# sajadn/Exemplar-VAE

Measured on AMD Instinct MI355X. Metric: training images/sec, higher is better.
Workload: dtype f32

## Files before the change

exemplar-vae_amd/csrc/evae_dense.hip:

```cpp

#include "evae_gemm_x6.h"
#include "evae_gemm_p6.h"
#include "evae_thin.h"
#include "evae_u8_prepare.h"

namespace evae {

__global__ void gated_bwd_input_kernel(const float* __restrict__ dout, const float* __restrict__ gout,
                                       const float* __restrict__ s, int M, int N, int ldo,
                                       float* __restrict__ dh, float* __restrict__ dg, int ldd) {
  const size_t n = (size_t)M * N;
  size_t i = (size_t)blockIdx.x * blockDim.x + threadIdx.x;
  const size_t stride = (size_t)gridDim.x * blockDim.x;
  for (; i < n; i += stride) {
    const size_t row = i / N, col = i % N;
    const float d = dout[row * (size_t)ldd + col], ov = gout[i], sv = s[i];
    const size_t o = row * (size_t)ldo + col;
    dh[o] = d * sv;
    dg[o] = d * ov * (1.0f - sv);
  }
}

__global__ __launch_bounds__(256) void gated_bwd_input_v4_kernel(const float4* __restrict__ dout, const float4* __restrict__ gout,
                                                                 const float4* __restrict__ s, unsigned nquads, unsigned nq,
// ... 953 lines not shown
  const bool narrow = gemm_x6_pick_bn(M, K) == 64;
  if (u8_img) {
    if (narrow) return launch_gemm_p6<EPI_GATE_BWD_IMG, 64, true>(g, 1, stream, "dense_bwd_data(p6, gate, byte-layer images)");
    return launch_gemm_p6<EPI_GATE_BWD_IMG, 128, true>(g, 1, stream, "dense_bwd_data(p6, gate, byte-layer images)");
  }
  if (gate) {
    if (narrow) return launch_gemm_p6<EPI_GATE_BWD, 64, true>(g, 1, stream, "dense_bwd_data(p6, gate)");
    return launch_gemm_p6<EPI_GATE_BWD, 128, true>(g, 1, stream, "dense_bwd_data(p6, gate)");
  }
  if (narrow) return launch_gemm_p6<EPI_LINEAR, 64, true>(g, 1, stream, "dense_bwd_data(p6)");
  return launch_gemm_p6<EPI_LINEAR, 128, true>(g, 1, stream, "dense_bwd_data(p6)");
}

struct P6WgradPlan { int kc, nz, ksplit, local; };
static P6WgradPlan p6_wgrad_plan(int nks, int N, int K, bool with_db) {
  P6WgradPlan p;
  p.kc = K + (with_db ? 1 : 0);
  const int tiles = cdiv(N, BM) * cdiv(p.kc, 64);
  static int slots = -1, local = -1;
  if (slots < 0) { const char* e = getenv("EVAE_P6_WGRAD_SLOTS"); slots = e ? atoi(e) : 256; }
  if (local < 0) { const char* e = getenv("EVAE_P6_WGRAD_LOCAL"); local = e ? atoi(e) : 16; }
  int nz = std::max(1, std::min(slots / std::max(tiles, 1), nks / 8));
  p.local = 0;
  if (local >= 8 && nz >= 8) {
    const int want = (local >= 16 && tiles * 2 <= 64 && nks / 16 >= 8) ? 16 : 8;
    if (tiles * (want / 8) <= 64) { nz = want; p.local = 1; }
  }
  p.ksplit = cdiv(nks, nz);
  p.nz = cdiv(nks, p.ksplit);
  return p;
}
extern "C" size_t evae_dense_bwd_weight_p6_workspace_bytes(int nks, int N, int K) {
  if (nks <= 0 || N <= 0 || K <= 0) return 256;
  const P6WgradPlan p = p6_wgrad_plan(nks, N, K, true);
  return align_up((size_t)p.nz * N * p.kc * sizeof(float), 256) + 256;
}
extern "C" int evae_dense_bwd_weight_p6(const void* dyT_img, const void* xT_img, int nks, int N, int K, float* dw, float* db,
                                        void* ws, size_t ws_bytes, evae_stream_t stream_) {
  EVAE_REQUIRE(nks > 0 && N > 0 && K > 0 && dyT_img && xT_img && dw, "dense_bwd_weight_p6: bad arguments");
  const P6WgradPlan p = p6_wgrad_plan(nks, N, K, db != nullptr);
  if (ws == nullptr || ws_bytes < (size_t)p.nz * N * p.kc * sizeof(float)) { set_error("dense_bwd_weight_p6: workspace too small (%zu)", ws_bytes); return EVAE_EWORKSPACE; }
  hipStream_t stream = (hipStream_t)stream_;
  GemmArgs g = {};
  g.ones_col = -1; g.npairs = 1;
  g.A[0] = (const float*)dyT_img; g.B[0] = (const float*)xT_img; g.Kc[0] = nks * P6_KS; g.M = N; g.N = p.kc;
  g.out0 = (float*)ws; g.ldo = p.kc; g.ksplit = p.ksplit; g.sk_local = p.local ? p.nz : 0;
  int rc = launch_gemm_p6<EPI_RAW, 64>(g, p.nz, stream, "dense_bwd_weight(p6)");
  if (rc) return rc;
  FinishArgs f = {};
  f.part = (const float*)ws; f.nz = p.nz; f.M = N; f.N = p.kc; f.ldo = p.kc; f.epi = EPI_RAW; f.out0 = dw;
  f.ones_col = db ? K : -1; f.out_db = db;
  return launch_finish(f, stream);
}
```

exemplar-vae_amd/csrc/evae_gemm_p6.h:

```cpp
#pragma once
#include "evae_gemm_kernel.h"

namespace evae {

typedef __bf16 p6_bf16x8 __attribute__((ext_vector_type(8)));
typedef __bf16 p6_bf16x4 __attribute__((ext_vector_type(4)));
typedef __attribute__((address_space(3))) void* p6_lds_t;
typedef __attribute__((address_space(3))) p6_bf16x4* p6_lds4_t;

constexpr int P6_NS = 3;
constexpr int p6_stage_bytes(int bn) { return P6_TILE + 3 * bn * 32; }
constexpr int p6_lds_bytes(int bn) { return P6_NS * p6_stage_bytes(bn); }

typedef unsigned p6_u32x2 __attribute__((ext_vector_type(2)));
template <int OFF>
__device__ __forceinline__ p6_u32x2 p6_tr_read(unsigned lds_addr) {
  p6_u32x2 r;
  asm volatile("ds_read_b64_tr_b16 %0, %1 offset:%2" : "=v"(r) : "v"(lds_addr), "n"(OFF));
  return r;
}

template <int EPI, int BN_, bool TA = false>
__global__ __launch_bounds__(256) __attribute__((amdgpu_waves_per_eu(2, 2))) void gemm_p6_kernel(const GemmArgs g) {
  constexpr bool GATED = (EPI == EPI_GATED || EPI == EPI_RAW_GATED);
  static_assert(BN_ == 128 || (BN_ == 64 && !GATED), "column tile: 128, or 64 for narrow plain outputs");
  constexpr int NW = 4, MT = 2, NT = BN_ / 64;
  constexpr int SB = p6_stage_bytes(BN_), BOFF = P6_TILE, BPL = BN_ * 32;
  extern __shared__ __attribute__((aligned(16))) float smem[];
  char* const lds = reinterpret_cast<char*>(smem);
  const int ntiles = g.tiles_m * g.tiles_n;
  int tile, zs = blockIdx.z;
  if (g.sk_local > 0) {
    const int id = blockIdx.x, xcd = id & 7, slot = id >> 3;
    const int j = slot / ntiles;
    tile = slot - j * ntiles;
    zs = xcd + 8 * j;
    if (zs >= g.sk_local) return;
  } else {
    const int id = blockIdx.x, xcd = id & 7, slot = id >> 3;
    const int qq = ntiles >> 3, rr = ntiles & 7;
    tile = (xcd < rr ? xcd * (qq + 1) : rr * (qq + 1) + (xcd - rr) * qq) + slot;
  }
  const int tm = tile / g.tiles_n, tn = tile - tm * g.tiles_n;
  const int m0 = tm * BM;
  const int n0 = GATED ? tn * 64 : tn * BN_;
  const int tid = threadIdx.x, lane = tid & 63;
  const int wave = __builtin_amdgcn_readfirstlane(tid >> 6);
  const int wr = wave >> 1, wc = wave & 1, l31 = lane & 31, lh = lane >> 5;

  f32x16 acc[MT][NT];
#pragma unroll
  for (int i = 0; i < MT; ++i)
#pragma unroll
    for (int j = 0; j < NT; ++j)
#pragma unroll
      for (int r = 0; r < 16; ++r) acc[i][j][r] = 0.f;

  const int nks = g.Kc[0] / P6_KS;
  int s_begin = 0, s_end = nks;
  if (g.ksplit > 0) {
    s_begin = zs * g.ksplit;
    const int e = s_begin + g.ksplit;
    if (e < s_end) s_end = e;
  }
  const int nst = s_end - s_begin;

  const unsigned a_nms = TA ? (unsigned)g.lda[0] : 0u;
  const unsigned grp = (unsigned)nks * P6_GROUP;
  const char* const abase = reinterpret_cast<const char*>(g.A[0]) + (TA ? (size_t)tm * 8 * P6_GROUP : (size_t)tm * 8 * grp);
  const char* const bbase = reinterpret_cast<const char*>(g.B[0]) + (size_t)(GATED ? tn * 8 : tn * (BN_ / 16)) * grp;
  const rsrc_t rA = make_rsrc(abase, 0x7FFFFFFFu);
  const rsrc_t rB = make_rsrc(bbase, 0x7FFFFFFFu);
  const unsigned voff_a = TA ? 0u : (unsigned)lh * grp + (unsigned)l31 * 16u;
  const unsigned voff_b = (unsigned)lh * grp + (unsigned)l31 * 16u;
  const unsigned voff_ta = (unsigned)lh * P6_GROUP + (unsigned)((((l31 >> 1) ^ (4 * lh)) * 32) + (l31 & 1) * 16);

  constexpr int NPIECE = BN_ == 128 ? 6 : 5;
  auto issue_piece = [&](int ks, int b, int q) {
    const unsigned so = (unsigned)ks * (unsigned)P6_GROUP;
    char* const st = lds + b * SB;
    if (q < 3) {
      if constexpr (TA) {
        __builtin_amdgcn_raw_ptr_buffer_load_lds(rA, (p6_lds_t)(st + q * P6_PLANE + wave * 1024), 16, voff_ta,
                                                 (unsigned)ks * a_nms * (unsigned)P6_GROUP + wave * 2 * P6_GROUP + q * P6_CHUNK, 0, 0);
      } else {
        __builtin_amdgcn_raw_ptr_buffer_load_lds(rA, (p6_lds_t)(st + q * P6_PLANE + wave * 1024), 16, voff_a,
                                                 so + (unsigned)(2 * wave) * grp + q * P6_CHUNK, 0, 0);
      }
    } else if constexpr (BN_ == 128) {
      const int p = q - 3;
      __builtin_amdgcn_raw_ptr_buffer_load_lds(rB, (p6_lds_t)(st + BOFF + p * BPL + wave * 1024), 16, voff_b,
                                               so + (unsigned)(2 * wave) * grp + p * P6_CHUNK, 0, 0);
// ... 109 lines not shown
            EVAE_P6_SB;
          }
          if constexpr (ISSUE) {
            constexpr int stride = NMF / 6;
            if (j % stride == 1 && j / stride < NPIECE) issue_piece(s_begin + i + 3, bcur, j / stride);
            EVAE_P6_SB;
          }
        }
    __builtin_amdgcn_s_setprio(0);
  };
#undef EVAE_P6_SB

  constexpr std::integral_constant<int, 0> I0{};
  constexpr std::integral_constant<int, 1> I1{};
  constexpr std::integral_constant<int, 2> I2{};
  constexpr std::true_type T{};
  constexpr std::false_type F{};
  if (nst > 0) {
    issue(s_begin, 0);
    if (nst > 1) issue(s_begin + 1, 1);
    if (nst > 2) issue(s_begin + 2, 2);
    if (nst > 2) wait_steps(I2); else if (nst > 1) wait_steps(I1); else wait_steps(I0);
    __builtin_amdgcn_s_barrier();
    read_all(I0, 0);
    int i = 0, b = 0;
    auto adv = [&]() { ++i; b = b == P6_NS - 1 ? 0 : b + 1; };
    while (i + 4 < nst) {
      iter(I0, T, T, I1, i, b); adv();
      iter(I1, T, T, I1, i, b); adv();
    }
#pragma unroll
    for (int u = 0; u < 2; ++u) {
      if (i < nst) {
        if (i + 3 < nst) iter(I0, T, T, I1, i, b);
        else if (i + 2 < nst) iter(I0, T, F, I1, i, b);
        else if (i + 1 < nst) iter(I0, T, F, I0, i, b);
        else iter(I0, F, F, I0, i, b);
        adv();
      }
      if (i < nst) {
        if (i + 3 < nst) iter(I1, T, T, I1, i, b);
        else if (i + 2 < nst) iter(I1, T, F, I1, i, b);
        else if (i + 1 < nst) iter(I1, T, F, I0, i, b);
        else iter(I1, F, F, I0, i, b);
        adv();
      }
    }
    __syncthreads();
  }
  if (g.dbg == 4) return;
  gemm_epilogue<EPI, BN_, NW, 0>(g, acc, m0, n0, tm, wr, wc, lane, smem, zs);
}

static __global__ __launch_bounds__(256) void p6_pack_rows_kernel(const float* __restrict__ x, const float* __restrict__ x2, int R, int K,
                                                           long long ld, int gated, int rows_img, int nks, unsigned char* __restrict__ img) {
  p6_pack_rows_element((size_t)blockIdx.x * blockDim.x + threadIdx.x, x, x2, R, K, ld, gated, rows_img, nks, img);
}

static __global__ __launch_bounds__(256) void p6_pack_cols_kernel(const float* __restrict__ x, const float* __restrict__ x2, int Kd, int R,
                                                           long long ld, int ones_row, int rows_img, int nks, unsigned char* __restrict__ img) {
  p6_pack_cols_element((size_t)blockIdx.x * blockDim.x + threadIdx.x, x, x2, Kd, R, ld, ones_row, rows_img, nks, img);
}

template <int EPI, int BN_ = 128, bool TA = false>
static int launch_gemm_p6(GemmArgs& g, int nz, hipStream_t stream, const char* what) {
  static bool attr_done = false;
  if (!attr_done) {
    (void)hipFuncSetAttribute((const void*)gemm_p6_kernel<EPI, BN_, TA>, hipFuncAttributeMaxDynamicSharedMemorySize, p6_lds_bytes(BN_));
    attr_done = true;
  }
  constexpr bool GATED = (EPI == EPI_GATED || EPI == EPI_RAW_GATED);
  g.tiles_m = cdiv(g.M, BM);
  g.tiles_n = cdiv(g.N, GATED ? 64 : BN_);
  dim3 grid(g.tiles_m * g.tiles_n, 1, nz);
  if (g.sk_local > 0) {
    if (g.sk_local != nz || g.ksplit <= 0) { set_error("%s: XCD-local split needs sk_local == nz and a split contraction", what); return EVAE_EINVAL; }
    grid = dim3(8 * cdiv(nz, 8) * g.tiles_m * g.tiles_n, 1, 1);
  }
  gemm_p6_kernel<EPI, BN_, TA><<<grid, 256, p6_lds_bytes(BN_), stream>>>(g);
  return check_launch(what);
}

}
```

exemplar-vae_amd/evae/_lib.py:

```python
import ctypes as C
import os

_HERE = os.path.dirname(os.path.abspath(__file__))
LIB_PATH = os.environ.get("EVAE_LIB_PATH") or os.path.join(os.path.dirname(_HERE), "csrc", "libevae_hip.so")

_p = C.c_void_p
_i = C.c_int
_f = C.c_float
_d = C.c_double
_z = C.c_size_t
_l = C.c_int64
_u = C.c_uint


class ConvDesc(C.Structure):
    _fields_ = [(n, C.c_int) for n in ("N", "C", "H", "W", "Co", "KH", "KW", "stride", "pad")]


class WtJob(C.Structure):
    _fields_ = [("w1", C.c_void_p), ("w2", C.c_void_p), ("dst", C.c_void_p), ("N", C.c_int), ("K", C.c_int), ("ldt", C.c_int)]


class CtlJob(C.Structure):
    _fields_ = [("stage0", C.c_void_p), ("stage1", C.c_void_p), ("ctl", C.c_void_p), ("bytes", C.c_size_t), ("state", C.c_void_p),
# ... 45 lines not shown
    "evae_mixture_lse_fwd_workspace_bytes": (_z, [_i, _i, _i]),
    "evae_mixture_lse_fwd": (_i, [_p, _i, _p, _p, _i, _i, _f, _p, _p, _p, _p, _z, _p]),
    "evae_mixture_lse_bwd_workspace_bytes": (_z, [_i, _i, _i]),
    "evae_mixture_lse_bwd": (_i, [_p, _i, _p, _p, _i, _i, _p, _p, _p, _p, _p, _p, _z, _p]),
    "evae_pseudo_inputs_fwd": (_i, [_p, _i, _i, _p, _p]),
    "evae_pseudo_inputs_bwd": (_i, [_p, _p, _i, _i, _p, _p]),
    "evae_pairdist_topk_workspace_bytes": (_z, [_i, _i, _i, _i]),
    "evae_pairdist_topk": (_i, [_p, _i, _p, _i, _i, _i, _u, _l, _p, _p, _p, _z, _p]),
    "evae_pairwise_distance": (_i, [_p, _i, _p, _i, _i, _p, _p]),
    "evae_topk_merge": (_i, [_p, _p, _i, _i, _i, _p, _p, _p]),
    "evae_select_exemplars": (_i, [_p, _i, _p, _i, _p, _p, _p, _p]),
    "evae_dense_fwd_workspace_bytes": (_z, [_i, _i, _i, _i]),
    "evae_gated_dense_fwd": (_i, [_p, _p, _i, _i, _i, _p, _p, _p, _p, _i, _p, _p, _p, _p, _z, _p]),
    "evae_linear_fwd": (_i, [_p, _p, _i, _i, _i, _p, _p, _i, _i, _f, _f, _p, _p, _p, _z, _p]),
    "evae_heads_reparam_fwd_workspace_bytes": (_z, [_i, _i, _i]),
    "evae_heads_reparam_fwd": (_i, [_p, _i, _i, _i, _p, _p, _p, _p, _i, _f, _f, _p, _p, _p, _p, _p, _p, _p, _z, _p]),
    "evae_heads_reparam_fwd_bcast_applies": (_i, [_i, _i, _i, _i]),
    "evae_heads_reparam_fwd_bcast": (_i, [_p, _i, _i, _i, _p, _p, _p, _p, _i, _f, _f, _p, _p, _p, _p, _p, _p, _p, _p, _i, _p]),
    "evae_heads_density_fwd": (_i, [_p, _i, _i, _i, _p, _p, _p, _p, _i, _f, _f, _p, _p, _p, _p, _p, _p, _z, _p]),
    "evae_log_normal_diag_bwd_hardtanh": (_i, [_p, _p, _p, _p, _f, _f, _p, _i, _i, _p, _p, _p, _p]),
    "evae_dense_bwd_data_wt_bytes": (_z, [_i, _i, _i]),
    "evae_dense_bwd_data_wt_ld": (_i, [_i]),
    "evae_dense_bwd_data_wt": (_i, [_p, _p, _p, _p, _i, _i, _i, _i, _p, _p, _p, _p, _i, _p, _p, _z, _p]),
    "evae_dense_bwd_data_workspace_bytes": (_z, [_i, _i, _i, _i]),
    "evae_dense_bwd_data": (_i, [_p, _p, _p, _p, _i, _i, _i, _i, _p, _p, _p, _p, _i, _p, _z, _p]),
    "evae_dense_bwd_weight_workspace_bytes": (_z, [_i, _i, _i]),
    "evae_dense_bwd_weight": (_i, [_p, _i, _i, _i, _p, _p, _i, _i, _p, _p, _i, _p, _z, _p]),
    "evae_dense_bwd_weight_phased": (_i, [_p, _i, _i, _i, _p, _p, _i, _i, _p, _p, _i, _p, _z, _i, _p]),
    "evae_dense_u8_supported": (_i, [_i, C.c_longlong]),
    "evae_dense_u8_prepared_bytes": (_z, [_i, _i]),
    "evae_dense_u8_prepare": (_i, [_p, _p, _i, _i, _p, _z, _p]),
    "evae_gated_dense_fwd_u8": (_i, [_p, _p, _i, _i, C.c_longlong, _f, _p, _p, _p, _i, _p, _p, _p]),
    "evae_dense_bwd_weight_u8_workspace_bytes": (_z, [_i, _i, _i]),
    "evae_dense_bwd_weight_u8": (_i, [_p, _i, _i, C.c_longlong, _p, _p, _i, C.c_longlong, _f, _p, _p, _p, _z, _p]),
    "evae_dense_bwd_weight_u8_phased": (_i, [_p, _i, _i, C.c_longlong, _p, _p, _i, C.c_longlong, _f, _p, _p, _p, _z, _i, _p]),
    "evae_dense_bwd_weight_u8_images": (_i, [_i, _i, _i, C.POINTER(C.c_size_t), C.POINTER(C.c_int)]),
    "evae_broadcast_scalar": (_i, [_p, _p, _i, _p]),
    "evae_sum_small": (_i, [_p, _i, _p, _p]),
    "evae_thin_configure": (_i, [_i]),
    "evae_p6_nks": (_i, [_i]),
    "evae_p6_nks_rows": (_i, [_i]),
    "evae_p6_image_bytes": (_z, [_i, _i]),
    "evae_gemm_p6_applies": (_i, [_i, _i, _i]),
    "evae_p6_pack_rows": (_i, [_p, _p, _i, _i, C.c_longlong, _i, _p, _z, _p]),
    "evae_p6_pack_cols": (_i, [_p, _p, _i, _i, C.c_longlong, _i, _i, _p, _z, _p]),
    "evae_p6_fill_row": (_i, [_p, _i, _i, _f, _i, _i, _p]),
    "evae_gated_dense_fwd_timg": (_i, [_p, _p, _i, _i, _i, _p, _p, _p, _p, _i, _p, _p, _p, _p, _i, _i, _i, _p, _z, _p]),
    "evae_gated_dense_fwd_u8_timg": (_i, [_p, _p, _i, _i, C.c_longlong, _f, _p, _p, _p, _i, _p, _p, _p, _i, _i, _i, _p]),
    "evae_dense_bwd_data_timg": (_i, [_p, _p, _p, _p, _i, _i, _i, _i, _p, _p, _p, _p, _i, _p, _p, _i, _i, _i, _p, _z, _p]),
    "evae_gated_dense_fwd_p6t": (_i, [_p, _i, _i, _i, _p, _p, _p, _i, _p, _p, _p]),
    "evae_dense_bwd_data_p6t": (_i, [_p, _i, _i, _i, _p, _i, _p, _p, _p, _p, _i, _p, _i, _i, _p]),
    "evae_dense_bwd_weight_p6_workspace_bytes": (_z, [_i, _i, _i]),
    "evae_dense_bwd_weight_p6": (_i, [_p, _p, _i, _i, _i, _p, _p, _p, _z, _p]),
    "evae_dense_bwd_data_img": (_i, [_p, _p, _p, _p, _i, _i, _i, _i, _p, _p, _p, _i, _i, _p, _p, _z, _p]),
    "evae_dense_bwd_weight_group": (_i, [_p, _i, _p]),
    "evae_dense_bwd_weight_finish_group": (_i, [_p, _i, _p]),
    "evae_gated_dense_bwd_input": (_i, [_p, _p, _p, _i, _i, _p, _p, _i, _p]),
    "evae_gated_dense_bwd_input_ld": (_i, [_p, _i, _p, _p, _i, _i, _p, _p, _i, _p]),
    "evae_gather_rows": (_i, [_p, _p, _p, _i, _i, _p, _p]),
    "evae_gated_dense_bwd": (_i, [_p, _i, _p, _p, _i, _i, _p, _p, _i, _p, _i, _p, _i, _p, _z, _p]),
    "evae_act_bwd": (_i, [_p, _p, _z, _i, _f, _f, _p, _p]),
    "evae_conv2d_workspace_bytes": (_z, [_p, _i, _i]),
    "evae_conv2d_fwd": (_i, [_p, _p, _p, _p, _p, _p, _i, _f, _f, _p, _p, _p, _p, _z, _p]),
    "evae_conv2d_bwd_data": (_i, [_p, _p, _p, _p, _p, _p, _p, _z, _p]),
    "evae_conv2d_bwd_weight": (_i, [_p, _p, _p, _p, _p, _p, _p, _z, _p]),
    "evae_conv2d_cl_supported": (_i, [_p, _i, _i]),
    "evae_conv2d_cl_dy_stride": (_i, [_i]),
    "evae_conv2d_cl_workspace_bytes": (_z, [_p, _i, _i]),
    "evae_conv2d_cl_fwd": (_i, [_p, _p, _p, _p, _p, _p, _i, _f, _f, _p, _p, _p, _p, _z, _p]),
    "evae_conv2d_cl_bwd_data": (_i, [_p, _p, _p, _p, _p, _p, _z, _p]),
    "evae_conv2d_cl_bwd_weight": (_i, [_p, _p, _p, _i, _p, _p, _p, _z, _p]),
    "evae_gemm_x6_configure": (_i, [_i, _i]),
    "evae_gemm_x6_applies": (_i, [_i, _i, _i]),
    "evae_elu_fwd": (_i, [_p, _z, _p, _p]),
    "evae_conv2d_cl_res_supported": (_i, [_p]),
    "evae_conv2d_cl_fwd_res": (_i, [_p, _p, _p, _p, _p, _p, _p, _z, _p]),
    "evae_conv2d_cl_bwd_data_res": (_i, [_p, _p, _p, _p, _p, _p, _p, _z, _p]),
    "evae_cw_image_bytes": (_z, [C.c_longlong, _i]),
    "evae_cw_supported": (_i, [_p, _i]),
    "evae_cw_workspace_bytes": (_z, [_p, _i]),
    "evae_cw_pack_image": (_i, [_p, _i, _i, _i, _i, _i, _p, _p]),
    "evae_cw_fwd_gated": (_i, [_p, _p, _p, _p, _p, _p, _p, _i, _p, _p, _p, _z, _p]),
    "evae_cw_bwd_data_gate": (_i, [_p, _i, _p, _p, _p, _p, _p, _p, _p, _p, _z, _p]),
    "evae_cw_gate_bwd_image": (_i, [_p, _p, _i, _p, _i, _i, _i, _i, _p, _p, _p]),
    "evae_cw_bwd_weight": (_i, [_p, _i, _p, _p, _p, _p, _p, _z, _p]),
    "evae_cw_res_supported": (_i, [_p]),
    "evae_cw_res_fwd": (_i, [_p, _p, _p, _p, _p, _p, _p, _p, _z, _p]),
    "evae_cw_res_bwd_data": (_i, [_p, _p, _p, _p, _p, _p, _p, _p, _z, _p]),
    "evae_cw_bwd_weight_plain": (_i, [_p, _p, _p, _p, _p, _p, _z, _p]),
    "evae_cw_first_fwd": (_i, [_p, _p, _p, _p, _p, _p, _p, _i, _p, _p, _p]),
    "evae_cw_first_workspace_bytes": (_z, []),
    "evae_cw_first_bwd_weight": (_i, [_p, _p, _p, _p, _p, _p, _z, _p]),
    "evae_cw_res_run_fwd": (_i, [_p, _i, _p, _p, _p, _p, _p, _p, _p]),
    "evae_cw_res_run_bwd": (_i, [_p, _i, _p, _p, _p, _p, _p, _p, _p, _p, _p, _z, _p]),
    "evae_cw_res_pack_filters": (_i, [_p, _i, _p, _p, _p, _p]),
    "evae_cw_plain_supported": (_i, [_p, _i]),
    "evae_cw_plain_workspace_bytes": (_z, [_p, _i]),
    "evae_cw_pack_image_ex": (_i, [_p, C.c_longlong, _i, _i, _p, C.c_longlong, _i, _i, _i, _i, _i, _p, _p]),
    "evae_cw_upsample2_bwd": (_i, [_p, C.c_longlong, _i, _i, _i, _i, _p, _p]),
    "evae_cw_plain_fwd": (_i, [_p, _p, _p, _p, _i, _p, _i, _p, _i, _p, _z, _p]),
    "evae_cw_plain_bwd_data": (_i, [_p, _i, _p, _p, _p, _i, _p, _p, _z, _p]),
    "evae_weight_norm_set_fwd": (_i, [_i, _p, _p, _p, _p, _p, _p]),
    "evae_weight_norm_set_bwd": (_i, [_i, _p, _p, _p, _p, _p, _p, _p, _p]),
    "evae_reparam_logq_fwd": (_i, [_p, _p, _p, _i, _i, _p, _p, _p]),
    "evae_reparam_logq_bwd": (_i, [_p, _p, _p, _p, _p, _p, _i, _i, _p, _p, _p]),
    "evae_reparam_logq_bwd_hardtanh": (_i, [_p, _p, _p, _p, _p, _p, _p, _p, _f, _f, _i, _i, _p, _p, _p]),
# ... 81 lines not shown
```

exemplar-vae_amd/evae/fused_vae.py:

```python
import ctypes as C
import os

import torch
import torch.distributed as dist

from . import _lib, handoff, ops, shard

ACT_NONE, ACT_SIGMOID, ACT_HARDTANH = ops.ACT_NONE, ops.ACT_SIGMOID, ops.ACT_HARDTANH

_STAGE_GEN = {}
_XT_GEN = {}
_ZEROED = {}
def node_merge(Cl, B):
    e = os.environ.get("EVAE_NODE_MERGE")
    if e is not None:
        return int(e)
    return 15 if Cl + B <= 8192 else 11


ONE_STREAM = [os.environ.get("EVAE_ONE_STREAM", "0") == "1"]
_APPROX_ROWS = {}

SCHED = int(os.environ.get("EVAE_SCHED", "0"))
FINISH_GROUP_HEAD = os.environ.get("EVAE_FINISH_GROUP_HEAD", "0") == "1"
# ... 528 lines not shown
        if sharded == 2:
            z_all, zi_all = ctx.dp
            RB = z_all.shape[0]
            lg = shard._all_gather_flat(torch.cat((lse.reshape(2, B), gp.reshape(1, B))))
            lse_all = torch.stack((lg[:, 0].reshape(-1), lg[:, 1].reshape(-1))).contiguous()
            gp_all = lg[:, 2].reshape(-1).contiguous()
            dz_all = torch.empty((RB, Z), **f32); dlv = torch.empty(Z, **f32)
            nb = lib.evae_prior_lse_bwd_workspace_bytes(RB, Cp, Z)
            w = k.ws("prior_bwd", nb)
            _lib.check(lib.evae_prior_lse_bwd(_vp(z_all), RB, _vp(centres_p), Cp, Z, _vp(lv_row), _vp(zi_all), _vp(ci), _vp(lse_all),
                                              _vp(gp_all), _vp(dz_all), _vp(dc_out), _vp(dlv), _vp(w), w.numel(), k.st),
                       "prior_bwd")
            dc_fold()
            dist.all_reduce(dz_all, op=dist.ReduceOp.SUM)
            r0 = dist.get_rank() * B
            dzp = dz_all[r0:r0 + B]
        elif prior_done:
            packed = ctx.prior_done[1]
            dzp = packed[:B * Z].view(B, Z); dlv = packed[B * Z:]
        else:
            assert ctx.prior_done is None, "fused vae step: the captured form's backward was called with another upstream gradient"
            packed = torch.empty(B * Z + Z, **f32)
            dzp = packed[:B * Z].view(B, Z); dlv = packed[B * Z:]
            nb = lib.evae_prior_lse_bwd_workspace_bytes(B, Cp, Z)
            w = k.ws("prior_bwd", nb)
            pb_args = (_vp(z), B, _vp(centres_p), Cp, Z, _vp(lv_row), _vp(zi), _vp(ci), _vp(lse), _vp(gp), _vp(dzp),
                       _vp(dc_out), _vp(dlv), _vp(w), w.numel())
            if sharded == 1 or dd_ is not None or not (SCHED & 1):
                _lib.check(lib.evae_prior_lse_bwd(*pb_args, k.st), "prior_bwd")
                dc_fold()
                if sharded == 1:
                    dist.all_reduce(packed, op=dist.ReduceOp.SUM)
                    if Cl > 0:
                        dmean_all[:Cl].mul_(float(dist.get_world_size()))
            else:
                _lib.check(lib.evae_prior_lse_bwd_phased(*pb_args, 1, k.st), "prior_bwd(1)")
                prior_finish = lambda: _lib.check(lib.evae_prior_lse_bwd_phased(*pb_args, 2, kd.st), "prior_bwd(2)")
        dz_ready = torch.cuda.Event(); dz_ready.record()
        if Cl > 0:
            if p6:
                nbh = lib.evae_dense_bwd_data_workspace_bytes(Cl, Z, H, 1)
                wh_ = k.ws("dgrad", nbh)
                flh = 2.0 * Cl * Z * H
                exh, pih = ops.gemm_pipe(Cl, H, False, flh)
                ops.probed("dense_bwd_data M=%d N=%d K=%d (gate-backward epilogue -> pre-split image)" % (Cl, Z, H), flh,
                           hbm_bytes=4.0 * Cl * (Z + 2 * H) + 6.0 * Cl * 2 * H, fn=
                           lambda: _lib.check(lib.evae_dense_bwd_data_timg(_vp(dmean_all), _vp(wm), None, None, Cl, Z, Z, H, _vp(A2), _vp(s2),
                                                                           None, None, 2 * H, _vp(None if ctx.wt is None else ctx.wt[0]),
                                                                           _vp(t_dq2), nks_m, 0, 0, _vp(wh_), wh_.numel(), k.st),
                                              "bwd_data_timg"))
            else:
                k.bwd_data(dmean_all, wm, None, None, Cl, Z, Z, H, A2, s2, dq2, dq2.data_ptr() + 4 * H, 2 * H,
                           wT=None if ctx.wt is None else ctx.wt[0])
            l2_dgrad(k, Cl, 0, 0)
        batch_rows_done = torch.cuda.Event()
        g_plv = gslot("plv", 1)
        g_wp = gslot("wp", D, H); g_bp = gslot("bp", D)
        g_d2 = gslot("d2", 2 * H, H); g_e2 = gslot("e2", 2 * H)
        g_d1 = gslot("d1", 2 * H, Z); g_e1 = gslot("e1", 2 * H)
        g_wl = gslot("wl", Z, H); g_bl = gslot("bl", Z)
        g_wm = gslot("wm", Z, H); g_bm = gslot("bm", Z)
        fin_group = FINISH_GROUP and data_ext.dtype == torch.uint8 and not (SCHED & 10) and Mp > 128 and not p6
        headw_early = bool(HEADW_EARLY and not fin_group and Cl > 0)
        with torch.cuda.stream(side):
            if not dpx_done:
                _lib.check(lib.evae_bernoulli_sigmoid_bwd(_vp(x), _vp(xmean), _vp(cRE), B, D, _vp(dpx), kd.st), "bernoulli_sigmoid_bwd")
            kd.bwd_data(dpx, wp, None, None, B, D, D, H, D2, sd2, dp2, dp2.data_ptr() + 4 * H, 2 * H)
            kd.bwd_data(dp2, d2h, dp2.data_ptr() + 4 * H, d2g, B, H, 2 * H, H, D1, sd1, dp1, dp1.data_ptr() + 4 * H, 2 * H)
            kd.bwd_data(dp1, d1h, dp1.data_ptr() + 4 * H, d1g, B, H, 2 * H, Z, None, None, dz, None, Z)
            side.wait_event(dz_ready)
            if prior_finish is not None:
                prior_finish()
            NODE_MERGE = node_merge(Cl, B)
            if NODE_MERGE & 12:
                RE_, logq_, logp_, loss_, KL_, means_ = ctx.elbo_keep if prior_done else (None,) * 6
                if prior_done and not (NODE_MERGE & 4):
                    _lib.check(lib.evae_elbo_assemble(_vp(logp_), _vp(RE_), _vp(logq_), _vp(beta_dev), 0.0 if beta_dev is not None else float(beta),
                                                      B, _vp(loss_), _vp(KL_), _vp(means_), kd.st), "elbo_assemble")
                    loss_ = None
                sum_here = bool(NODE_MERGE & 8)
                _lib.check(lib.evae_reparam_logq_bwd_hardtanh_tail(
                    _vp(z_mean), _vp(logvar), _vp(eps), _vp(z), _vp(dz), _vp(dzp), _vp(cKL), _vp(lv_pre), -6.0, 2.0, B, Z,
                    _vp(dmean_all.data_ptr() + off * Z), _vp(dlvp), _vp(logp_), _vp(RE_), _vp(logq_), _vp(beta_dev),
                    0.0 if beta_dev is not None else float(beta), _vp(loss_), _vp(KL_), _vp(means_),
                    _vp(dlv) if sum_here else None, Z, _vp(g_plv) if sum_here else None, kd.st), "reparam_bwd_tail")
            else:
                if prior_done:
                    RE_, logq_, logp_, loss_, KL_, means_ = ctx.elbo_keep
                    _lib.check(lib.evae_elbo_assemble(_vp(logp_), _vp(RE_), _vp(logq_), _vp(beta_dev), 0.0 if beta_dev is not None else float(beta),
                                                      B, _vp(loss_), _vp(KL_), _vp(means_), kd.st), "elbo_assemble")
                _lib.check(lib.evae_reparam_logq_bwd_hardtanh(_vp(z_mean), _vp(logvar), _vp(eps), _vp(z), _vp(dz), _vp(dzp), _vp(cKL),
                                                              _vp(lv_pre), -6.0, 2.0, B, Z, _vp(dmean_all.data_ptr() + off * Z),
                                                              _vp(dlvp), kd.st), "reparam_bwd")
            if headw_early:
                kd.bwd_weight(dmean_all, Mp, Z, Z, A2, None, H, H, g_wm, g_bm)
            if p6:
                nbh = lib.evae_dense_bwd_data_workspace_bytes(B, Z, H, 2)
                wh2 = kd.ws("dgrad", nbh)
                _lib.check(lib.evae_dense_bwd_data_timg(_vp(dmean_all.data_ptr() + off * Z), _vp(wm), _vp(dlvp), _vp(wl), B, Z, Z, H,
                                                        _vp(A2.data_ptr() + off * H), _vp(s2.data_ptr() + off * H),
                                                        _vp(dq2.data_ptr() + off * 2 * H), _vp(dq2.data_ptr() + off * 2 * H + 4 * H), 2 * H,
                                                        None, _vp(t_dq2), nks_m, 0, Cl, _vp(wh2), wh2.numel(), kd.st), "bwd_data_timg(batch)")
            else:
                kd.bwd_data(dmean_all.data_ptr() + off * Z, wm, dlvp, wl, B, Z, Z, H, A2.data_ptr() + off * H,
                            s2.data_ptr() + off * H, dq2.data_ptr() + off * 2 * H, dq2.data_ptr() + off * 2 * H + 4 * H, 2 * H)
            dq2_rows_done = torch.cuda.Event(); dq2_rows_done.record()
            l2_dgrad(kd, B, off, Cl)
            batch_rows_done.record()


        def leaves():
            with torch.cuda.stream(side):
                if fin_group and FINISH_GROUP_HEAD:
                    kd.bwd_weight(dmean_all, Mp, Z, Z, A2, None, H, H, g_wm, g_bm, phase=1, ws_name="wgradh")
                elif not headw_early:
                    kd.bwd_weight(dmean_all, Mp, Z, Z, A2, None, H, H, g_wm, g_bm)
                jobs = ((dpx, B, D, D, D2, H, H, g_wp, g_bp), (dp2, B, 2 * H, 2 * H, D1, H, H, g_d2, g_e2),
                        (dp1, B, 2 * H, 2 * H, z, Z, Z, g_d1, g_e1),
                        (dlvp, B, Z, Z, A2.data_ptr() + off * H, H, H, g_wl, g_bl))
                grouped = B <= 128 and GROUP_LEAVES and all(n_ % 4 == 0 and k_ % 4 == 0 for _, _, n_, _, _, k_, _, _, _ in jobs)
                if grouped:
                    arr = (_lib.WgradJob * len(jobs))()
                    for i_, (dy_, m_, n_, ldy_, x_, k_, ldx_, dw_, db_) in enumerate(jobs):
                        arr[i_].dy = dy_.data_ptr(); arr[i_].x = x_ if isinstance(x_, int) else x_.data_ptr()
                        arr[i_].dw = dw_.data_ptr(); arr[i_].db = db_.data_ptr()
                        arr[i_].M, arr[i_].N, arr[i_].K, arr[i_].ldy, arr[i_].ldx = m_, n_, k_, ldy_, ldx_
                    _lib.check(lib.evae_dense_bwd_weight_group(C.cast(arr, C.c_void_p), len(jobs), kd.st), "bwd_weight_group")
                else:
                    for dy_, m_, n_, ldy_, x_, k_, ldx_, dw_, db_ in jobs:
                        kd.bwd_weight(dy_, m_, n_, ldy_, x_, None, k_, ldx_, dw_, db_)
                if not (NODE_MERGE & 8):
                    _lib.check(lib.evae_sum_small(_vp(dlv), Z, _vp(g_plv), kd.st), "sum_small")
        leaves()
        split_wait = bool(SCHED & 256) and not (SCHED & 10)
        main.wait_event(dq2_rows_done if split_wait else batch_rows_done)
        g_w2 = gslot("w2", 2 * H, H); g_b2 = gslot("b2", 2 * H)
        w2_args = (dq2, Mp, 2 * H, 2 * H, A1, None, H, H, g_w2, g_b2)
        g_w1 = gslot("w1", 2 * H, D); g_b1 = gslot("b1", 2 * H)
        def w1_grad(no_finish=False):
            if data_ext.dtype == torch.uint8:
                nb = lib.evae_dense_bwd_weight_u8_workspace_bytes(Mp, 2 * H, D)
                w = k.ws("wgrad_u8_fused", nb)
                fl = 2.0 * Mp * 2 * H * D
                have_xt = ctx.xt is not None and ctx.xt == (w.data_ptr(), _XT_GEN.get(w.data_ptr()))
                ops.probed("dense_bwd_weight_u8 M=%d N=%d K=%d (uint8 rows, three bf16 terms; %s)"
                           % (Mp, 2 * H, D, "GEMM; planes summed by the step's last grouped launch" if no_finish else "pre-passes + GEMM + finish"),
                           fl, lambda: _lib.check(lib.evae_dense_bwd_weight_u8_phased(_vp(dq1), Mp, 2 * H, 2 * H, _vp(data_ext), _vp(rows), D,
                                                                                      ldd, 1.0 / 255.0, _vp(g_w1), _vp(g_b1), _vp(w),
                                                                                      w.numel(), (4 if have_xt else 0) | (16 if no_finish else 0), k.st)
                                              if (have_xt or no_finish) else
                                              lib.evae_dense_bwd_weight_u8(_vp(dq1), Mp, 2 * H, 2 * H, _vp(data_ext), _vp(rows), D,
                                                                           ldd, 1.0 / 255.0, _vp(g_w1), _vp(g_b1), _vp(w),
                                                                           w.numel(), k.st), "bwd_weight_u8"),
                           executed=3 * fl, pipe="bf16-mfma")
            else:
                k.bwd_weight(dq1, Mp, 2 * H, 2 * H, data_ext, rows, D, ldd, g_w1, g_b1)
        if SCHED & 2:
            k.bwd_weight(*w2_args, phase=1, ws_name="wgrad2")
            w2_done = torch.cuda.Event(); w2_done.record()
            w1_grad()
            with torch.cuda.stream(side):
                side.wait_event(w2_done)
                k.bwd_weight(*w2_args, phase=2, ws_name="wgrad2", finish_on=kd)
        elif (SCHED & 8) and data_ext.dtype == torch.uint8:
            nb = lib.evae_dense_bwd_weight_u8_workspace_bytes(Mp, 2 * H, D)
            w = k.ws("wgrad_u8_fused", nb)

            def w1_phase(phase, st):
                _lib.check(lib.evae_dense_bwd_weight_u8_phased(_vp(dq1), Mp, 2 * H, 2 * H, _vp(data_ext), _vp(rows), D, ldd, 1.0 / 255.0,
                                                               _vp(g_w1), _vp(g_b1), _vp(w), w.numel(), phase, st), "bwd_weight_u8_phased")
            dq1_ready = torch.cuda.Event(); dq1_ready.record()
            with torch.cuda.stream(side):
                side.wait_event(dq1_ready)
                w1_phase(1, kd.st)
                pre_done = torch.cuda.Event(); pre_done.record()
            k.bwd_weight(*w2_args)
            main.wait_event(pre_done)
            w1_phase(2, k.st)
        elif fin_group:
            k.bwd_weight(*w2_args, phase=1, ws_name="wgrad2")
            if split_wait:
                main.wait_event(batch_rows_done)
            w1_grad(no_finish=True)
            if FINISH_GROUP_HEAD:
                main.wait_stream(side)
            arr = (_lib.WgradFinishJob * 3)()
            w_u8 = k.ws("wgrad_u8_fused", lib.evae_dense_bwd_weight_u8_workspace_bytes(Mp, 2 * H, D))
            w_2 = ops._workspace("wgrad2" + k.sfx, lib.evae_dense_bwd_weight_workspace_bytes(Mp, 2 * H, H), dev)
            w_h = ops._workspace("wgradh" + kd.sfx, lib.evae_dense_bwd_weight_workspace_bytes(Mp, Z, H), dev)
            fjobs = ((1, Mp, 2 * H, D, 2 * H, ldd, 1.0 / 255.0, g_w1, g_b1, w_u8), (0, Mp, 2 * H, H, 2 * H, H, 1.0, g_w2, g_b2, w_2),
                     (0, Mp, Z, H, Z, H, 1.0, g_wm, g_bm, w_h))[:3 if FINISH_GROUP_HEAD else 2]
            for i_, (byte_, m_, n_, k_, ldy_, ldx_, xs_, dw_, db_, ws_) in enumerate(fjobs):
                arr[i_].byte_rows, arr[i_].M, arr[i_].N, arr[i_].K, arr[i_].ldy, arr[i_].ldx = byte_, m_, n_, k_, ldy_, ldx_
                arr[i_].x_scale = xs_; arr[i_].dw = dw_.data_ptr(); arr[i_].db = db_.data_ptr()
                arr[i_].ws = ws_.data_ptr(); arr[i_].ws_bytes = ws_.numel()
            _lib.check(lib.evae_dense_bwd_weight_finish_group(C.cast(arr, C.c_void_p), len(fjobs), k.st), "bwd_weight_finish_group")
        elif p6:
            nbw = lib.evae_dense_bwd_weight_p6_workspace_bytes(nks_m, 2 * H, H)
            ww = k.ws("wgrad_p6", nbw)
            flw = 2.0 * Mp * 2 * H * H
            ops.probed("dense_bwd_weight M=%d N=%d K=%d (+db; pre-split bf16 images, split-K GEMM + finish)" % (Mp, 2 * H, H), flw,
                       lambda: _lib.check(lib.evae_dense_bwd_weight_p6(_vp(t_dq2), _vp(t_h1), nks_m, 2 * H, H, _vp(g_w2), _vp(g_b2), _vp(ww),
                                                                       ww.numel(), k.st), "bwd_weight_p6"), executed=6 * flw, pipe="bf16-mfma")
            if split_wait:
                main.wait_event(batch_rows_done)
            w1_grad()
        else:
            k.bwd_weight(*w2_args)
            if split_wait:
                main.wait_event(batch_rows_done)
            w1_grad()
        main.wait_stream(side)
        ctx.bufs = None
        ctx.elbo_keep = None
        ctx.prior_done = None
        ctx.dd = None
        grads = (g_plv, g_wp, g_bp, g_w1[:H], g_b1[:H], g_w1[H:], g_b1[H:], g_w2[:H], g_b2[:H], g_w2[H:], g_b2[H:],
                 g_wm, g_bm, g_wl, g_bl, g_d1[:H], g_e1[:H], g_d1[H:], g_e1[H:], g_d2[:H], g_e2[:H], g_d2[H:], g_e2[H:])
        return (None,) * 15 + grads
```

include/evae_hip.h:

```cpp
#ifndef EVAE_HIP_H
#define EVAE_HIP_H

#include <stddef.h>
#include <stdint.h>

#ifdef __cplusplus
extern "C" {
#endif

#define EVAE_OK 0
#define EVAE_EINVAL (-1)
#define EVAE_EWORKSPACE (-2)
#define EVAE_ELAUNCH (-3)

#define EVAE_ABI_VERSION 1

typedef void* evae_stream_t;

int evae_version(void);
const char* evae_last_error(void);
int evae_ctl_upload(void* d_stage, const void* h_pinned, void* d_ctl, size_t bytes, evae_stream_t up, evae_stream_t step,
                    void* ev_used, void* ev_up);

int evae_host_dedup(const int64_t* draws, int n_draws, int64_t n_rows, int cap, int64_t* rows, int64_t* inv, int64_t* rep, float* mult);
// ... 245 lines not shown
                          float* dmu, float* dlogvar, evae_stream_t stream);
int evae_reparam_logq_bwd_hardtanh(const float* mu, const float* logvar, const float* eps, const float* z,
                                   const float* dz, const float* dz2, const float* dlogq, const float* lv_pre,
                                   float lo, float hi, int B, int zdim, float* dmu, float* dlv_pre,
                                   evae_stream_t stream);
int evae_reparam_logq_bwd_hardtanh_tail(const float* mu, const float* logvar, const float* eps, const float* z, const float* dz,
                                        const float* dz2, const float* dlogq, const float* lv_pre, float lo, float hi, int B,
                                        int zdim, float* dmu, float* dlv_pre, const float* logp, const float* RE,
                                        const float* logq, const float* beta_dev, float beta_host, float* loss, float* KL,
                                        float* means, const float* sum_src, int sum_n, float* sum_dst, evae_stream_t stream);
int evae_log_normal_diag_fwd(const float* x, const float* mu, const float* logvar, int B, int zdim,
                             float* out, evae_stream_t stream);
int evae_log_normal_diag_bwd(const float* x, const float* mu, const float* logvar, const float* dout,
                             int B, int zdim, float* dx, float* dmu, float* dlogvar,
                             evae_stream_t stream);
int evae_elbo_fwd(const float* RE, const float* logq, const float* logp, const float* beta_dev,
                  float beta_host, int B, float* loss, float* KL, float* means, evae_stream_t stream);
int evae_elbo2_fwd(const float* RE, const float* logq1, const float* logp1, const float* logq2, const float* logp2,
                   const float* beta_dev, float beta_host, int B, float* loss, float* KL, float* means, evae_stream_t stream);
int evae_elbo_bwd(const float* dloss, int n_dloss, const float* dRE, int n_dRE, const float* dKL, int n_dKL,
                  const float* beta_dev, float beta_host, int B, float* cRE, float* cKL, float* neg_cKL,
                  evae_stream_t stream);
int evae_step_stats_add(const float* loss, const float* re, const float* kl, float* step3, float* totals3,
                        evae_stream_t stream);
int evae_thin_configure(int max_rows);
int evae_p6_nks(int K);
int evae_p6_nks_rows(int M);
size_t evae_p6_image_bytes(int rows, int nks);
int evae_gemm_p6_applies(int M, int N, int gated);
int evae_p6_pack_rows(const float* x, const float* x2 , int R, int K, long long ld, int gated, void* img,
                      size_t img_bytes, evae_stream_t stream);
int evae_p6_pack_cols(const float* x, const float* x2 , int Kd, int R, long long ld, int ones_row ,
                      int nks, void* img, size_t img_bytes, evae_stream_t stream);
int evae_p6_fill_row(void* img, int nks, int row, float value, int k_begin, int k_end, evae_stream_t stream);
int evae_gated_dense_fwd_timg(const float* x, const int64_t* rows, int M, int K, int ldx, const float* wh, const float* bh,
                              const float* wg, const float* bg, int N, float* out, float* save_h, float* save_s,
                              void* timg, int t_nks, int t_row0, int t_kbase, void* ws, size_t ws_bytes, evae_stream_t stream);
int evae_gated_dense_fwd_u8_timg(const unsigned char* x, const int64_t* rows, int M, int K, long long ldx, float x_scale,
                                 const void* prepared, const float* bh, const float* bg, int N, float* out, float* save_s,
                                 void* timg, int t_nks, int t_row0, int t_kbase, evae_stream_t stream);
int evae_dense_bwd_data_timg(const float* dy1, const float* w1, const float* dy2, const float* w2, int M, int N, int ldy, int K,
                             const float* out_prev, const float* s_prev, float* dx_or_dh, float* dg, int ldo,
                             const float* wT , void* timg, int t_nks, int t_row0, int t_kbase, void* ws,
                             size_t ws_bytes, evae_stream_t stream);
int evae_gated_dense_fwd_p6t(const void* xT_img, int x_nks, int M, int K, const void* w_img, const float* bh, const float* bg,
                             int N, float* out , float* save_s , evae_stream_t stream);
int evae_dense_bwd_data_p6t(const void* dyT_img, int dy_nks, int M, int N, const void* wT_img, int K, const float* out_prev,
                            const float* s_prev, float* dh, float* dg, int ldo, void* u8_img, int u8_nslab, int u8_mbase,
                            evae_stream_t stream);
size_t evae_dense_bwd_weight_p6_workspace_bytes(int nks, int N, int K);
int evae_dense_bwd_weight_p6(const void* dyT_img, const void* xT_img, int nks, int N, int K, float* dw ,
                             float* db , void* ws, size_t ws_bytes,
                             evae_stream_t stream);
int evae_broadcast_scalar(const float* src, float* dst, int n, evae_stream_t stream);
int evae_sum_small(const float* x, int n, float* out, evae_stream_t stream);
int evae_batch_prologue(const float* data, int64_t ldd, const int64_t* idx, int B, int D, int binarize,
                        const int64_t* seed_ctr , float* x_out, int64_t ldx,
                        float* eps_out , int zdim, evae_stream_t stream);
int evae_batch_prologue_u8(const unsigned char* data, int64_t ldd, const int64_t* idx, int B, int D, int binarize,
                           const int64_t* seed_ctr, float x_div, float* x_out, int64_t ldx, unsigned char* stage, int64_t lds,
                           float* eps_out, int zdim, evae_stream_t stream);
typedef struct { const float* w1; const float* w2; float* dst; int N, K, ldt; } evae_wt_job_t;
int evae_batch_prologue_u8_prepare(const unsigned char* data, int64_t ldd, const int64_t* idx, int B, int D, int binarize,
                                   const int64_t* seed_ctr, float x_div, float* x_out, int64_t ldx, unsigned char* stage,
                                   int64_t lds, float* eps_out, int zdim, const float* wh, const float* wg, int N, int K,
                                   void* prepared, size_t prepared_bytes, const evae_wt_job_t* jobs, int njobs,
                                   evae_stream_t stream);
typedef struct { const void* stage0; const void* stage1; void* ctl; size_t bytes; const int* state; size_t idx_word, seed_word; } evae_ctl_job_t;
typedef struct { const float* x; const float* x2; void* img; size_t img_bytes; long long ld; int cols, R, K, flag, nks; } evae_p6_pack_job_t;
int evae_batch_prologue_u8_step(const unsigned char* data, int64_t ldd, int B, int D, int binarize, float x_div, float* x_out,
                                int64_t ldx, unsigned char* stage, int64_t lds, float* eps_out, int zdim, const float* wh,
                                const float* wg, int N, int K, void* prepared, size_t prepared_bytes, const evae_wt_job_t* jobs,
                                int njobs, const evae_ctl_job_t* ctl, const evae_p6_pack_job_t* packs, int npacks,
                                evae_stream_t stream);
int evae_log_normal_diag_bwd_hardtanh(const float* x, const float* mu, const float* logvar, const float* lv_pre, float lo, float hi,
                                      const float* dout, int B, int zdim, float* dx, float* dmu, float* dlv_pre, evae_stream_t stream);
int evae_bernoulli_ll_fwd(const float* x, const float* mean, int B, int D, float* out,
                          evae_stream_t stream);
int evae_bernoulli_ll_bwd(const float* x, const float* mean, const float* dout, int B, int D,
                          float* dmean, evae_stream_t stream);
int evae_log_logistic256_fwd(const float* x, const float* mean, const float* logvar, int lv_scalar, int B, int D,
                             float* out , evae_stream_t stream);
int evae_log_logistic256_bwd(const float* x, const float* mean, const float* logvar, int lv_scalar,
                             const float* dout , int B, int D, float* dmean, float* dlogvar,
                             float* ws_rows , evae_stream_t stream);
int evae_bernoulli_sigmoid_bwd(const float* x, const float* mean, const float* dout, int B, int D,
                               float* dpre, evae_stream_t stream);
int evae_bernoulli_unit_step(const float* x, const float* mean, int B, int D, const float* beta_dev, float beta_host, float* RE,
                             float* cRE, float* cKL, float* neg_cKL, float* dpre, evae_stream_t stream);

typedef struct {
  float* param;
  const float* grad;
  float* exp_avg;
  float* exp_avg_sq;
  int64_t numel;
} evae_adam_tensor_t;
size_t evae_adam_normgrad_workspace_bytes(int n_tensors);
int evae_adam_normgrad_step(const evae_adam_tensor_t* tensors , int n_tensors,
                            int64_t max_numel, int step, double lr, double beta1, double beta2, double eps,
                            double weight_decay, const float* step_size_dev ,
                            void* ws, size_t ws_bytes, evae_stream_t stream);
int evae_adam_normgrad_step_stats(const evae_adam_tensor_t* tensors , int n_tensors, int64_t max_numel, int step,
                                  double lr, double beta1, double beta2, double eps, double weight_decay,
                                  const float* step_size_dev, void* ws, size_t ws_bytes, const float* loss, const float* re,
                                  const float* kl, float* step3, float* totals3, int* toggle, evae_stream_t stream);
// ... 6 lines not shown
```

Measured before the change: 194,700.

## Fuse layer-2 data-gradient and weight-gradient GEMMs into one paired launch

Refactors the p6 GEMM kernel into a device body and adds a pair kernel that runs the dense backward-data GEMM (with gate-backward epilogue writing bf16 images) and the split-K weight-gradient GEMM in a single launch, partitioned by block index. The Python p6 path calls the combined entry point instead of a separate l2_dgrad plus weight-grad launch. It also re-plans the split-K slice count to use more slices and drops the split wait for p6. This is meant to cut launch overhead and fill the GPU better with two moderately sized GEMMs. The cost is that both halves share the larger LDS size and occupancy settings, and the data GEMM now has to wait until the batch rows are done.

```diff
diff --git a/exemplar-vae_amd/csrc/evae_dense.hip b/exemplar-vae_amd/csrc/evae_dense.hip
--- a/exemplar-vae_amd/csrc/evae_dense.hip
+++ b/exemplar-vae_amd/csrc/evae_dense.hip
@@ -1029,3 +1029,62 @@
   f.ones_col = db ? K : -1; f.out_db = db;
   return launch_finish(f, stream);
 }
+
+constexpr int P6_PAIR_SLICES = 32;
+static P6WgradPlan p6_wgrad_pair_plan(int nks, int N, int K, bool with_db, int slices) {
+  P6WgradPlan p = p6_wgrad_plan(nks, N, K, with_db);
+  if (slices < 0) return p;
+  int nz = slices;
+  if (nz == 0) {
+    if (!p.local) return p;
+    nz = std::max(p.nz, std::min(P6_PAIR_SLICES, nks / 8));
+  }
+  nz = std::max(1, std::min(nz, nks));
+  p.ksplit = cdiv(nks, nz);
+  p.nz = cdiv(nks, p.ksplit);
+  return p;
+}
+extern "C" int evae_dense_bwd_data_weight_p6t_plan(int nks, int N, int K, int with_db, int slices, int* nz, int* ksplit) {
+  EVAE_REQUIRE(nks > 0 && N > 0 && K > 0 && nz && ksplit, "dense_bwd_data_weight_p6t_plan: bad arguments");
+  const P6WgradPlan p = p6_wgrad_pair_plan(nks, N, K, with_db != 0, slices);
+  *nz = p.nz; *ksplit = p.ksplit;
+  return EVAE_OK;
+}
+extern "C" size_t evae_dense_bwd_data_weight_p6t_workspace_bytes(int nks, int N, int K, int slices) {
+  if (nks <= 0 || N <= 0 || K <= 0) return 256;
+  const P6WgradPlan p = p6_wgrad_pair_plan(nks, N, K, true, slices);
+  return align_up((size_t)p.nz * N * p.kc * sizeof(float), 256) + 256;
+}
+extern "C" int evae_dense_bwd_data_weight_p6t(const void* dyT_img, int nks, int M, int N, const void* wT_img, int K,
+                                              const float* out_prev, const float* s_prev, void* u8_img, int u8_nslab, int u8_mbase,
+                                              const void* xT_img, float* dw, float* db, void* ws, size_t ws_bytes, int slices,
+                                              evae_stream_t stream_) {
+  EVAE_REQUIRE(M > 0 && K > 0 && N > 0 && nks >= cdiv(M, 128) * 8, "dense_bwd_data_weight_p6t: bad sizes M=%d N=%d K=%d (k-steps %d)",
+               M, N, K, nks);
+  EVAE_REQUIRE(dyT_img && wT_img && xT_img && dw && out_prev && s_prev && u8_img && (u8_mbase % 8) == 0,
+               "dense_bwd_data_weight_p6t: bad arguments");
+  const P6WgradPlan p = p6_wgrad_pair_plan(nks, N, K, db != nullptr, slices);
+  if (ws == nullptr || ws_bytes < (size_t)p.nz * N * p.kc * sizeof(float)) {
+    set_error("dense_bwd_data_weight_p6t: workspace too small (%zu)", ws_bytes); return EVAE_EWORKSPACE;
+  }
+  hipStream_t stream = (hipStream_t)stream_;
+  GemmArgs a = {};
+  a.ones_col = -1; a.npairs = 1;
+  a.A[0] = (const float*)dyT_img; a.lda[0] = nks; a.B[0] = (const float*)wT_img; a.Kc[0] = p6_nks(N) * P6_KS;
+  a.M = M; a.N = K; a.e0 = out_prev; a.e1 = s_prev;
+  a.img = (unsigned short*)u8_img; a.img_nslab = u8_nslab; a.img_mbase = u8_mbase;
+  GemmArgs b = {};
+  b.ones_col = -1; b.npairs = 1;
+  b.A[0] = (const float*)dyT_img; b.B[0] = (const float*)xT_img; b.Kc[0] = nks * P6_KS; b.M = N; b.N = p.kc;
+  b.out0 = (float*)ws; b.ldo = p.kc; b.ksplit = p.ksplit; b.sk_local = p.nz > 1 ? p.nz : 0;
+  int rc;
+  if (gemm_x6_pick_bn(M, K) == 64)
+    rc = launch_gemm_p6_pair<EPI_GATE_BWD_IMG, 64, true, EPI_RAW, 64, false>(a, b, p.nz, stream, "dense_bwd_data_weight(p6 pair)");
+  else
+    rc = launch_gemm_p6_pair<EPI_GATE_BWD_IMG, 128, true, EPI_RAW, 64, false>(a, b, p.nz, stream, "dense_bwd_data_weight(p6 pair)");
+  if (rc) return rc;
+  FinishArgs f = {};
+  f.part = (const float*)ws; f.nz = p.nz; f.M = N; f.N = p.kc; f.ldo = p.kc; f.epi = EPI_RAW; f.out0 = dw;
+  f.ones_col = db ? K : -1; f.out_db = db;
+  return launch_finish(f, stream);
+}
diff --git a/exemplar-vae_amd/csrc/evae_gemm_p6.h b/exemplar-vae_amd/csrc/evae_gemm_p6.h
--- a/exemplar-vae_amd/csrc/evae_gemm_p6.h
+++ b/exemplar-vae_amd/csrc/evae_gemm_p6.h
@@ -20,24 +20,23 @@
   return r;
 }
 
-template <int EPI, int BN_, bool TA = false>
-__global__ __launch_bounds__(256) __attribute__((amdgpu_waves_per_eu(2, 2))) void gemm_p6_kernel(const GemmArgs g) {
+template <int EPI, int BN_, bool TA>
+__device__ __forceinline__ void gemm_p6_body(const GemmArgs& g, const int bid, const int zslice, float* const smem) {
   constexpr bool GATED = (EPI == EPI_GATED || EPI == EPI_RAW_GATED);
   static_assert(BN_ == 128 || (BN_ == 64 && !GATED), "column tile: 128, or 64 for narrow plain outputs");
   constexpr int NW = 4, MT = 2, NT = BN_ / 64;
   constexpr int SB = p6_stage_bytes(BN_), BOFF = P6_TILE, BPL = BN_ * 32;
-  extern __shared__ __attribute__((aligned(16))) float smem[];
   char* const lds = reinterpret_cast<char*>(smem);
   const int ntiles = g.tiles_m * g.tiles_n;
-  int tile, zs = blockIdx.z;
+  int tile, zs = zslice;
   if (g.sk_local > 0) {
-    const int id = blockIdx.x, xcd = id & 7, slot = id >> 3;
+    const int id = bid, xcd = id & 7, slot = id >> 3;
     const int j = slot / ntiles;
     tile = slot - j * ntiles;
     zs = xcd + 8 * j;
     if (zs >= g.sk_local) return;
   } else {
-    const int id = blockIdx.x, xcd = id & 7, slot = id >> 3;
+    const int id = bid, xcd = id & 7, slot = id >> 3;
     const int qq = ntiles >> 3, rr = ntiles & 7;
     tile = (xcd < rr ? xcd * (qq + 1) : rr * (qq + 1) + (xcd - rr) * qq) + slot;
   }
@@ -253,6 +252,25 @@
   gemm_epilogue<EPI, BN_, NW, 0>(g, acc, m0, n0, tm, wr, wc, lane, smem, zs);
 }
 
+template <int EPI, int BN_, bool TA = false>
+__global__ __launch_bounds__(256) __attribute__((amdgpu_waves_per_eu(2, 2))) void gemm_p6_kernel(const GemmArgs g) {
+  extern __shared__ __attribute__((aligned(16))) float smem[];
+  gemm_p6_body<EPI, BN_, TA>(g, (int)blockIdx.x, (int)blockIdx.z, smem);
+}
+
+template <int EPI_A, int BN_A, bool TA_A, int EPI_B, int BN_B, bool TA_B>
+__global__ __launch_bounds__(256) __attribute__((amdgpu_waves_per_eu(2, 2))) void gemm_p6_pair_kernel(const GemmArgs a, const GemmArgs b,
+                                                                                                   const int blocks_a) {
+  extern __shared__ __attribute__((aligned(16))) float smem[];
+  const int id = blockIdx.x;
+  if (id < blocks_a) {
+    if (id >= a.tiles_m * a.tiles_n) return;
+    gemm_p6_body<EPI_A, BN_A, TA_A>(a, id, 0, smem);
+  } else {
+    gemm_p6_body<EPI_B, BN_B, TA_B>(b, id - blocks_a, 0, smem);
+  }
+}
+
 static __global__ __launch_bounds__(256) void p6_pack_rows_kernel(const float* __restrict__ x, const float* __restrict__ x2, int R, int K,
                                                            long long ld, int gated, int rows_img, int nks, unsigned char* __restrict__ img) {
   p6_pack_rows_element((size_t)blockIdx.x * blockDim.x + threadIdx.x, x, x2, R, K, ld, gated, rows_img, nks, img);
@@ -282,4 +300,26 @@
   return check_launch(what);
 }
 
-}
+template <int EPI_A, int BN_A, bool TA_A, int EPI_B, int BN_B, bool TA_B>
+static int launch_gemm_p6_pair(GemmArgs& a, GemmArgs& b, int nz_b, hipStream_t stream, const char* what) {
+  constexpr int LDS = p6_lds_bytes(BN_A) > p6_lds_bytes(BN_B) ? p6_lds_bytes(BN_A) : p6_lds_bytes(BN_B);
+  static bool attr_done = false;
+  if (!attr_done) {
+    (void)hipFuncSetAttribute((const void*)gemm_p6_pair_kernel<EPI_A, BN_A, TA_A, EPI_B, BN_B, TA_B>,
+                              hipFuncAttributeMaxDynamicSharedMemorySize, LDS);
+    attr_done = true;
+  }
+  constexpr bool GATED_A = (EPI_A == EPI_GATED || EPI_A == EPI_RAW_GATED), GATED_B = (EPI_B == EPI_GATED || EPI_B == EPI_RAW_GATED);
+  if (a.sk_local != 0 || a.ksplit != 0) { set_error("%s: the first GEMM of a pair is not split", what); return EVAE_EINVAL; }
+  if (nz_b > 1 ? (b.sk_local != nz_b || b.ksplit <= 0) : (b.sk_local != 0)) {
+    set_error("%s: the second GEMM of a pair is un-split or XCD-local", what); return EVAE_EINVAL;
+  }
+  a.tiles_m = cdiv(a.M, BM); a.tiles_n = cdiv(a.N, GATED_A ? 64 : BN_A);
+  b.tiles_m = cdiv(b.M, BM); b.tiles_n = cdiv(b.N, GATED_B ? 64 : BN_B);
+  const int blocks_a = cdiv(a.tiles_m * a.tiles_n, 8) * 8;
+  const int blocks_b = (b.sk_local > 0 ? 8 * cdiv(nz_b, 8) : 1) * b.tiles_m * b.tiles_n;
+  gemm_p6_pair_kernel<EPI_A, BN_A, TA_A, EPI_B, BN_B, TA_B><<<dim3(blocks_a + blocks_b, 1, 1), 256, LDS, stream>>>(a, b, blocks_a);
+  return check_launch(what);
+}
+
+}
diff --git a/exemplar-vae_amd/evae/_lib.py b/exemplar-vae_amd/evae/_lib.py
--- a/exemplar-vae_amd/evae/_lib.py
+++ b/exemplar-vae_amd/evae/_lib.py
@@ -121,6 +121,9 @@
     "evae_dense_bwd_data_p6t": (_i, [_p, _i, _i, _i, _p, _i, _p, _p, _p, _p, _i, _p, _i, _i, _p]),
     "evae_dense_bwd_weight_p6_workspace_bytes": (_z, [_i, _i, _i]),
     "evae_dense_bwd_weight_p6": (_i, [_p, _p, _i, _i, _i, _p, _p, _p, _z, _p]),
+    "evae_dense_bwd_data_weight_p6t_plan": (_i, [_i, _i, _i, _i, _i, C.POINTER(C.c_int), C.POINTER(C.c_int)]),
+    "evae_dense_bwd_data_weight_p6t_workspace_bytes": (_z, [_i, _i, _i, _i]),
+    "evae_dense_bwd_data_weight_p6t": (_i, [_p, _i, _i, _i, _p, _i, _p, _p, _p, _i, _i, _p, _p, _p, _p, _z, _i, _p]),
     "evae_dense_bwd_data_img": (_i, [_p, _p, _p, _p, _i, _i, _i, _i, _p, _p, _p, _i, _i, _p, _p, _z, _p]),
     "evae_dense_bwd_weight_group": (_i, [_p, _i, _p]),
     "evae_dense_bwd_weight_finish_group": (_i, [_p, _i, _p]),
diff --git a/exemplar-vae_amd/evae/fused_vae.py b/exemplar-vae_amd/evae/fused_vae.py
--- a/exemplar-vae_amd/evae/fused_vae.py
+++ b/exemplar-vae_amd/evae/fused_vae.py
@@ -604,7 +604,8 @@
             else:
                 k.bwd_data(dmean_all, wm, None, None, Cl, Z, Z, H, A2, s2, dq2, dq2.data_ptr() + 4 * H, 2 * H,
                            wT=None if ctx.wt is None else ctx.wt[0])
-            l2_dgrad(k, Cl, 0, 0)
+            if not p6:
+                l2_dgrad(k, Cl, 0, 0)
         batch_rows_done = torch.cuda.Event()
         g_plv = gslot("plv", 1)
         g_wp = gslot("wp", D, H); g_bp = gslot("bp", D)
@@ -684,7 +685,7 @@
                 if not (NODE_MERGE & 8):
                     _lib.check(lib.evae_sum_small(_vp(dlv), Z, _vp(g_plv), kd.st), "sum_small")
         leaves()
-        split_wait = bool(SCHED & 256) and not (SCHED & 10)
+        split_wait = bool(SCHED & 256) and not (SCHED & 10) and not p6
         main.wait_event(dq2_rows_done if split_wait else batch_rows_done)
         g_w2 = gslot("w2", 2 * H, H); g_b2 = gslot("b2", 2 * H)
         w2_args = (dq2, Mp, 2 * H, 2 * H, A1, None, H, H, g_w2, g_b2)
@@ -748,14 +749,15 @@
                 arr[i_].ws = ws_.data_ptr(); arr[i_].ws_bytes = ws_.numel()
             _lib.check(lib.evae_dense_bwd_weight_finish_group(C.cast(arr, C.c_void_p), len(fjobs), k.st), "bwd_weight_finish_group")
         elif p6:
-            nbw = lib.evae_dense_bwd_weight_p6_workspace_bytes(nks_m, 2 * H, H)
+            nbw = lib.evae_dense_bwd_data_weight_p6t_workspace_bytes(nks_m, 2 * H, H, 0)
             ww = k.ws("wgrad_p6", nbw)
-            flw = 2.0 * Mp * 2 * H * H
-            ops.probed("dense_bwd_weight M=%d N=%d K=%d (+db; pre-split bf16 images, split-K GEMM + finish)" % (Mp, 2 * H, H), flw,
-                       lambda: _lib.check(lib.evae_dense_bwd_weight_p6(_vp(t_dq2), _vp(t_h1), nks_m, 2 * H, H, _vp(g_w2), _vp(g_b2), _vp(ww),
-                                                                       ww.numel(), k.st), "bwd_weight_p6"), executed=6 * flw, pipe="bf16-mfma")
-            if split_wait:
-                main.wait_event(batch_rows_done)
+            flw = 2.0 * Cl * 2 * H * H + 2.0 * Mp * 2 * H * H
+            ops.probed("dense_bwd_pair: data M=%d N=%d+%d K=%d + weight M=%d N=%d K=%d (+db) (pre-split bf16 images, one launch; "
+                       "gate-backward epilogue -> bf16 tile images; split-K finish)" % (Cl, H, H, H, Mp, 2 * H, H), flw,
+                       lambda: _lib.check(lib.evae_dense_bwd_data_weight_p6t(
+                           _vp(t_dq2), nks_m, Cl, 2 * H, _vp(w2t_img), H, _vp(A1), _vp(s1), _vp(img_ptr), nslab_img.value, 0,
+                           _vp(t_h1), _vp(g_w2), _vp(g_b2), _vp(ww), ww.numel(), 0, k.st), "bwd_data_weight_p6t"),
+                       executed=6 * flw, pipe="bf16-mfma")
             w1_grad()
         else:
             k.bwd_weight(*w2_args)
diff --git a/include/evae_hip.h b/include/evae_hip.h
--- a/include/evae_hip.h
+++ b/include/evae_hip.h
@@ -321,6 +321,12 @@
 int evae_dense_bwd_weight_p6(const void* dyT_img, const void* xT_img, int nks, int N, int K, float* dw ,
                              float* db , void* ws, size_t ws_bytes,
                              evae_stream_t stream);
+int evae_dense_bwd_data_weight_p6t_plan(int nks, int N, int K, int with_db, int slices, int* nz, int* ksplit);
+size_t evae_dense_bwd_data_weight_p6t_workspace_bytes(int nks, int N, int K, int slices);
+int evae_dense_bwd_data_weight_p6t(const void* dyT_img, int nks, int M, int N, const void* wT_img, int K, const float* out_prev,
+                                   const float* s_prev, void* u8_img, int u8_nslab, int u8_mbase, const void* xT_img,
+                                   float* dw , float* db , void* ws, size_t ws_bytes, int slices,
+                                   evae_stream_t stream);
 int evae_broadcast_scalar(const float* src, float* dst, int n, evae_stream_t stream);
 int evae_sum_small(const float* x, int n, float* out, evae_stream_t stream);
 int evae_batch_prologue(const float* data, int64_t ldd, const int64_t* idx, int B, int D, int binarize,
```

New measurement: 192,200. 0.987x the previous value.
